# Meng-333/SRADSGAN

Measured on AMD Instinct MI355X. Metric: training images/sec (216x216, x4), higher is better.
Workload: dtype f32 (split-bf16 products: 3 bf16 MFMA terms per fp32 multiply, fp32 accumulate)

## Files before the change

### sradsgan_amd/csrc/conv_dev.h

```cpp
#pragma once
#include "conv_internal.h"

namespace srhip {

typedef unsigned int u32x4 __attribute__((ext_vector_type(4)));
typedef unsigned int u32x2 __attribute__((ext_vector_type(2)));
constexpr int FBK = 16;
constexpr int FLS = FBK + 4;
constexpr unsigned F_OOB = 0x80000000u;

struct FastGeom {
  int N, Hs, Ws, C, lds;
  int OH, OW, M;
  int ss;
  int TH, TW, dh0, dhs, dw0, dws;
  int kh0, khs, kw0, kws, KW;
  int Hd, Wd, dsd, ph, pw, ldd, K;
  int ldw, ldr;
  float slope;
  int flags, accumulate, dst_identity;
  unsigned src_bytes, w_bytes;
  int src_pp = 0, dst_pp = 0, src_guard = 0, dst_guard = 0;
  unsigned src_plane_bytes = 0, dst_plane_bytes = 0;
  void* dst2_pp = nullptr;
  int dst2_guard = 0;
  const float* res2 = nullptr;
  const float* res3 = nullptr;
};
struct ResRequest {
  const float* r2 = nullptr;
  const float* r3 = nullptr;
  int served = 0;
};
extern thread_local ResRequest g_res_req;
struct SignRequest {
  void* words = nullptr;
  size_t bytes = 0;
  int mode = 0;
  int served = 0;
};
extern thread_local SignRequest g_sign_req;
long pp_sign_tiles(int n, int h, int w, int cout);
struct PhaseSet {
  int n = 0;
  int first[5] = {0, 0, 0, 0, 0};
  struct P {
    int ph, pw, OH, OW, kh0, kw0, TH, TW, dh0, dw0, M, nblk_m;
  } p[4];
};
struct PhaseRequest {
  PhaseSet ps;
  int active = 0, launched = 0;
};
extern thread_local PhaseRequest g_phase_req;
struct Dst2Request {
  void* pp = nullptr;
  int served = 0;
};
extern thread_local Dst2Request g_dst2_req;

}
extern int g_tail_dbg;
namespace srhip {
extern int g_fast_cfg;
extern int g_wgrad_cfg;
extern int g_fast_dynlds;
extern int g_fast_ablate;
extern int g_sgam_cfg;
extern int g_pers_grid;
extern int g_pers_abl;
extern int g_rowtap_addr;
extern int g_rowtap_pipe;
extern int g_patch_ks;
extern int g_pers_small;
extern int g_flat_blocks;
extern int g_flat_abl;
extern int g_flat_f32_k8;
extern int g_patch8;
extern int g_patch8_abl;
extern int g_phase_batch;
extern int g_headconv_rows;
extern int g_pool_epi_any;

enum FastCfg : int {
  FAST_CFG_FORCE_PATCH = -2,
  FAST_CFG_FORCE_DMA = -1,
  FAST_CFG_AUTO = 0,
  FAST_CFG_REG_128x128_K32 = 1,
  FAST_CFG_REG_64x128 = 2,
  FAST_CFG_REG_64x128_K32 = 3,
  FAST_CFG_REG_256x128 = 4,
  FAST_CFG_REG_128x128 = 5,
  FAST_CFG_REG_128x64_K32 = 6,
  FAST_CFG_REG_64x64 = 7,
  FAST_CFG_REG_128x64_4x1_K32 = 8,
  FAST_CFG_REG_ONLY = 20,
  FAST_CFG_NO_PATCH = 21,
  FAST_CFG_NO_VALU = 22,
  FAST_CFG_PATCH_TO_DMA = 23,
  FAST_CFG_PATCH_NARROW = 24,
};
inline bool fast_cfg_allows_dma(int cfg) { return cfg < 1 || cfg == FAST_CFG_PATCH_TO_DMA || cfg == FAST_CFG_PATCH_NARROW; }

enum WgradCfg : int {
  WGRAD_CFG_AUTO = 0,
  WGRAD_CFG_BN64 = 1,
  WGRAD_CFG_BN128 = 2,
  WGRAD_CFG_BK32 = 3,
  WGRAD_CFG_BK32_BN64 = 4,
  WGRAD_CFG_TILE256 = 5,
  WGRAD_CFG_SCALAR_REDUCE_GENERIC = 6,
  WGRAD_CFG_NO_ROWTAP = 7,
  WGRAD_CFG_SCALAR_REDUCE = 8,
  WGRAD_CFG_NO_PAIRED_TAILS = 9,
  WGRAD_CFG_REG = 10,
  WGRAD_CFG_ROWTAP_TARGET = 100,
};

constexpr int FAST_EPI_MASK = 0x3f;
constexpr int FAST_ABL_NO_LOADS = 0x100;
constexpr int FAST_ABL_NO_BARRIER = 0x200;
constexpr int FAST_ABL_TIMING = FAST_ABL_NO_LOADS | FAST_ABL_NO_BARRIER;
constexpr int FAST_ABL_PLAIN_STORES = 0x400;

inline bool bytes_ok(long pixels, int ld, int c, unsigned* out) {
  const long b = pixels > 0 ? ((pixels - 1) * (long)ld + c) * 4L : 0;
  if (b >= (1L << 31)) return false;
  *out = (unsigned)b;
  return true;
}

__device__ inline float4 bufload4(__amdgpu_buffer_rsrc_t r, unsigned byte_off) {
  u32x4 v = __builtin_amdgcn_raw_buffer_load_b128(r, byte_off, 0, 0);
  return __builtin_bit_cast(float4, v);
}

__device__ inline f32x16 mfma32f(float a, float b, f32x16 c) {
  return __builtin_amdgcn_mfma_f32_32x32x2f32(a, b, c, 0, 0, 0);
}

__device__ inline int xcd_tile(int b, int nblk) {
  const int q = nblk >> 3, r = nblk & 7, x = b & 7;
  return (x < r ? x * (q + 1) : r * (q + 1) + (x - r) * q) + (b >> 3);
}

typedef __bf16 bf16x8_t __attribute__((ext_vector_type(8)));

__device__ inline void split_bf16x8(const float4& v0, const float4& v1, bf16x8_t& hi, bf16x8_t& lo) {
  const float v[8] = {v0.x, v0.y, v0.z, v0.w, v1.x, v1.y, v1.z, v1.w};
#pragma unroll
  for (int j = 0; j < 8; ++j) {
    const __bf16 h = (__bf16)v[j];
    hi[j] = h;
    lo[j] = (__bf16)(v[j] - (float)h);
  }
}

typedef _Float16 f16x8_t __attribute__((ext_vector_type(8)));
template <int PROD>
__device__ __forceinline__ f32x16 mma16(const bf16x8_t& a, const bf16x8_t& b, const f32x16& c) {
  if constexpr (PROD == 2)
    return __builtin_amdgcn_mfma_f32_32x32x16_f16(__builtin_bit_cast(f16x8_t, a), __builtin_bit_cast(f16x8_t, b), c, 0, 0, 0);
  else
    return __builtin_amdgcn_mfma_f32_32x32x16_bf16(a, b, c, 0, 0, 0);
}
template <int PROD>
__device__ __forceinline__ bf16x8_t round16x8(const float4& v0, const float4& v1) {
  const float v[8] = {v0.x, v0.y, v0.z, v0.w, v1.x, v1.y, v1.z, v1.w};
  if constexpr (PROD == 2) {
    f16x8_t h;
#pragma unroll
    for (int j = 0; j < 8; ++j) h[j] = (_Float16)v[j];
    return __builtin_bit_cast(bf16x8_t, h);
  } else {
    bf16x8_t h;
#pragma unroll
    for (int j = 0; j < 8; ++j) h[j] = (__bf16)v[j];
    return h;
  }
}
template <int PROD>
constexpr int nprod() { return PROD == 0 ? 3 : 1; }

__device__ inline void lds_dma16(const float* gsrc, unsigned lds_dst_uniform) {
  unsigned keep;
  asm volatile(
      "s_mov_b32 %0, m0\n\ts_mov_b32 m0, %2\n\ts_nop 0\n\tglobal_load_lds_dwordx4 %1, off\n\ts_mov_b32 m0, %0"
      : "=&s"(keep)
      : "v"(gsrc), "s"(lds_dst_uniform)
      : "memory");
}

__device__ inline void lds_dma16_buf(unsigned voff, __amdgpu_buffer_rsrc_t r, unsigned lds_dst_uniform) {
  asm volatile("s_mov_b32 m0, %2\n\ts_nop 0\n\tbuffer_load_dwordx4 %0, %1, 0 offen lds" ::"v"(voff), "s"(r), "s"(lds_dst_uniform) : "memory");
}

struct PatchGeom {
  int PH, PW, tiles_h, tiles_w;
  int PWP, PR, npieces;
  int lo_h, lo_w;
  unsigned gmap;
};

template <int N>
__device__ inline void wait_vmcnt() {
  asm volatile("s_waitcnt vmcnt(%0)" ::"n"(N) : "memory");
}

template <int I>
struct IC {
  static constexpr int value = I;
};

__device__ __forceinline__ void patch_pixel(int r, int PH, int PW, unsigned gmap, int& orow, int& ocol) {
  const int a = PW >> 4, b = PW & 15;
  const int grp = (gmap >> (4 * (r >> 4))) & 15, j = r & 15;
  const int nfull = PH * a;
  if (grp < nfull) {
    orow = grp / a;
    ocol = (grp - orow * a) * 16 + j;
  } else if (b > 0) {
    const int idx = (grp - nfull) * 16 + j;
    orow = idx / b;
    ocol = 16 * a + (idx - orow * b);
    if (orow >= PH) { orow = PH; ocol = 0; }
  } else {
    orow = PH;
    ocol = 0;
  }
}

struct PoolRequest {
  float* out = nullptr;
  unsigned sec_bytes = 0;
  int served_nseg = 0;
};
extern thread_local PoolRequest g_pool_req;
int launch_patch_pers(const float* src, const float* wt, const float* bias, const float* residual, const float* actmask,
                      float* dst, const FastGeom& g, const PatchGeom& pg, int nbm, int nbn, bool wide, int prod, int eflags,
                      hipStream_t st);

int launch_patch8(const float* src, const float* wt, const float* bias, const float* actmask, float* dst, const FastGeom& g,
                  const PatchGeom& pg, int nbm, int eflags, hipStream_t st);

}
```

### sradsgan_amd/csrc/conv_fast_fprop.hip

```cpp
#include "conv_dev.h"

namespace srhip {

int g_fast_ablate = 0;


template <int BM, int BN, int WM, int WN, int BK, int MATH = 0>
__global__ __launch_bounds__(WM* WN * 64) void fast_conv_kernel(const float* __restrict__ src,
                                                                 const float* __restrict__ wt,
                                                                 const float* __restrict__ bias,
                                                                 const float* __restrict__ residual,
                                                                 const float* __restrict__ rowscale,
                                                                 const float* __restrict__ chanscale,
                                                                 const float* __restrict__ actmask,
                                                                 float* __restrict__ dst, FastGeom g, int nblk_m,
                                                                 int nblk_n) {
  constexpr int NT = WM * WN * 64;
  constexpr int WTM = BM / WM, WTN = BN / WN;
  constexpr int TM = WTM / 32, TN = WTN / 32;
  constexpr int LS = BK + 4;
  constexpr int QPR = BK / 4;
  constexpr int RPP = NT / QPR;
  constexpr int AR = (BM + RPP - 1) / RPP, BR = (BN + RPP - 1) / RPP;
  constexpr int STAGE = (BM + BN) * LS;
// ... 1352 lines not shown
      r.wide = g.K >= 128;
      r.nbn = cdiv(g.K, r.wide ? 128 : 64);
      r.try_patch8 = r.wide && !a.residual;
      r.try_pers = true;
    }
    return r;
  }
  const bool valu_ok = cfg != FAST_CFG_REG_ONLY && cfg != FAST_CFG_NO_VALU &&
                       !(g.flags & ~(SRHIP_EPI_BIAS | SRHIP_EPI_LRELU | SRHIP_EPI_GRADDATA)) && !g.accumulate;
  if (g.K <= 4 && valu_ok && g.TH == 3 && g.TW == 3 && g.ss == 1 && g.dsd == 1 && g.ph == 0 && g.pw == 0 && g.Hd == g.OH && g.Wd == g.OW &&
      (g.dhs == 1 || g.dhs == -1) && (g.dws == 1 || g.dws == -1) && g.M >= 65536) {
    r.family = FpropFamily::Narrow;
    r.nd = g.K == 3 ? 3 : 4;
    return r;
  }
  if (g.K == 1 && g.C % 4 == 0 && g.lds % 4 == 0 && aligned16(a.src) && aligned16(a.wt) && g.M < 65536 && valu_ok) {
    r.family = FpropFamily::Dot;
    return r;
  }
  const int math16 = g_conv_math == 2 ? ((g.flags & SRHIP_EPI_GRADDATA) ? 2 : 3) : 1;
  if (g.K <= 32) {
    static const RegLaunch small[4] = {launch_reg<128, 32, 4, 1, 16>, launch_reg<128, 32, 4, 1, 16, 1>, launch_reg<128, 32, 4, 1, 16, 2>,
                                       launch_reg<128, 32, 4, 1, 16, 3>};
    r.family = FpropFamily::Reg;
    if (g_conv_math >= 1 && cfg != FAST_CFG_REG_ONLY && !(g.flags & (SRHIP_EPI_CHANSCALE | FAST_ABL_TIMING))) r.math = math16;
    r.reg = small[r.math];
    return r;
  }
  const bool al16 = g.K % 4 == 0 && g.ldd % 4 == 0 && aligned16(a.dst) && (!a.residual || (g.ldr % 4 == 0 && aligned16(a.residual))) &&
                    aligned16(a.actmask) && aligned16(a.bias);
  const bool dma_ok = fast_cfg_allows_dma(cfg) && !(g.flags & FAST_ABL_TIMING) && g.K >= 64 && al16;
  bool patch_to_dma = false;
  if (dma_ok && g_conv_math >= 1 && cfg != FAST_CFG_NO_PATCH && !scaled_a && !g.accumulate && plan_patch(g, &r.pg)) {
    r.nbm = g.N * r.pg.tiles_h * r.pg.tiles_w;
    r.wide = g.K >= 128 && cfg != FAST_CFG_PATCH_NARROW;
    r.bn = r.wide ? 128 : 64;
    r.nbn = cdiv(g.K, r.bn);
    const bool enough = (long)r.nbm * r.nbn >= 256;
    if (cfg == FAST_CFG_PATCH_TO_DMA) {
      patch_to_dma = enough;
    } else if (enough || cfg == FAST_CFG_FORCE_PATCH) {
      r.family = FpropFamily::Patch;
      r.math = math16;
      r.try_pers = !(g.flags & FAST_ABL_PLAIN_STORES);
      r.try_patch8 = r.try_pers && r.wide && math16 == 1 && !a.residual;
      r.ks = math16 == 1 && !r.wide && g_patch_ks && g.C % 32 == 0 && g.C >= 32;
      r.epi = math16 != 1 ? -1 : epi_variant(r.eflags, false);
      if (r.ks && r.epi != 0 && r.epi != SRHIP_EPI_BIAS && r.epi != SRHIP_EPI_RESIDUAL) r.epi = -1;
      return r;
    }
  }
  if (dma_ok && (!(r.eflags & SRHIP_EPI_CHANSCALE) || aligned16(a.chanscale))) {
    r.nbm = cdiv(g.M, 128);
    const bool force = cfg == FAST_CFG_FORCE_DMA || patch_to_dma;
    const long min_tiles = g_conv_math >= 1 ? 128 : 512;
    r.wide = g.K >= 128 && ((long)r.nbm * cdiv(g.K, 128) >= min_tiles || force);
    if (r.wide || (long)r.nbm * cdiv(g.K, 64) >= min_tiles || force) {
      r.family = FpropFamily::Dma;
      r.bn = r.wide ? 128 : 64;
      r.nbn = cdiv(g.K, r.bn);
      r.math = g_conv_math >= 1 ? math16 : 0;
      r.epi = (r.math >= 2 || g.accumulate) ? -1 : epi_variant(r.eflags, true);
      return r;
    }
  }
  struct Forced { int cfg; bool k128, k32; RegLaunch fn; };
  static const Forced forced[] = {
      {FAST_CFG_REG_128x128_K32, true, true, launch_reg<128, 128, 2, 2, 32>}, {FAST_CFG_REG_64x128, true, false, launch_reg<64, 128, 1, 4, 16>},
      {FAST_CFG_REG_64x128_K32, true, true, launch_reg<64, 128, 1, 4, 32>},   {FAST_CFG_REG_256x128, true, false, launch_reg<256, 128, 4, 2, 16>},
      {FAST_CFG_REG_128x128, true, false, launch_reg<128, 128, 2, 2, 16>},    {FAST_CFG_REG_128x64_K32, false, true, launch_reg<128, 64, 2, 2, 32>},
      {FAST_CFG_REG_64x64, false, false, launch_reg<64, 64, 2, 2, 16>},       {FAST_CFG_REG_128x64_4x1_K32, false, true, launch_reg<128, 64, 4, 1, 32>}};
  r.family = FpropFamily::Reg;
  const long b128 = (long)cdiv(g.M, 128) * cdiv(g.K, 128), b64 = (long)cdiv(g.M, 128) * cdiv(g.K, 64);
  r.reg = (g.K >= 128 && b128 >= 512) ? launch_reg<128, 128, 2, 2, 16> : b64 >= 512 ? launch_reg<128, 64, 2, 2, 16> : launch_reg<64, 64, 2, 2, 16>;
  for (const Forced& c : forced)
    if (cfg == c.cfg && (!c.k128 || g.K >= 128) && (!c.k32 || g.C % 32 == 0)) r.reg = c.fn;
  return r;
}

template <int BN, int EPI, int PROD = 0>
static int launch_patch(const ConvOperands& a, const FastGeom& g, const FpropRoute& r, hipStream_t st) {
  hipLaunchKernelGGL((conv_patch_kernel<BN, EPI, PROD>), dim3(r.nbm * r.nbn), dim3(256), 0, st, a.src, weight_section(a, g, PROD + 1), a.bias,
                     a.residual, a.actmask, a.dst, g, r.pg, r.nbm, r.nbn);
  return check_launch("conv_patch");
}
template <int EPI>
static int launch_patch_ks(const ConvOperands& a, const FastGeom& g, const FpropRoute& r, hipStream_t st) {
  hipLaunchKernelGGL((conv_patch_ks_kernel<EPI>), dim3(r.nbm * r.nbn), dim3(256), 0, st, a.src, weight_section(a, g, 1), a.bias, a.residual,
                     a.actmask, a.dst, g, r.pg, r.nbm, r.nbn);
  return check_launch("conv_patch_ks");
}
template <int BN, int EPI, int MATH>
static int launch_dma(const ConvOperands& a, const FastGeom& g, const FpropRoute& r, hipStream_t st) {
  PhaseSet ps;
  int grid = r.nbm * r.nbn;
  if constexpr (MATH <= 1) {
    if (g.dst2_pp) g_dst2_req.served = 1;
    if (g_phase_req.active) {
      ps = g_phase_req.ps;
      grid = 0;
      for (int k = 0; k < ps.n; ++k) {
        ps.first[k] = grid;
        grid += ps.p[k].nblk_m * r.nbn;
      }
      ps.first[ps.n] = grid;
      g_phase_req.launched = 1;
    }
  }
  hipLaunchKernelGGL((fast_conv_dma_kernel<128, BN, EPI, MATH>), dim3(grid), dim3(256), g_fast_dynlds, st, a.src, weight_section(a, g, MATH),
                     a.bias, a.residual, a.rowscale, a.chanscale, a.actmask, a.dst, g, r.nbm, r.nbn, ps);
  return check_launch("fast_conv_dma");
}
template <bool TAIL, class F>
static int with_epi(int epi, F f) {
  switch (epi) {
    case 0: return f(IC<0>{});
    case 1: return f(IC<1>{});
    case 3: return f(IC<3>{});
    case 32: return f(IC<32>{});
    case 4: return f(IC<4>{});
    case 29: if constexpr (TAIL) return f(IC<29>{}); [[fallthrough]];
    default: return f(IC<-1>{});
  }
}

static int launch_fprop(const ConvOperands& a, const FastGeom& g, const FpropRoute& r, hipStream_t st) {
  const bool wide = r.bn == 128;
  switch (r.family) {
    case FpropFamily::Nothing:
      return SRHIP_OK;
    case FpropFamily::Planes:
    case FpropFamily::Patch: {
      if (r.try_patch8) {
        const int rc8 = launch_patch8(a.src, a.wt, a.bias, a.actmask, a.dst, g, r.pg, r.nbm, r.eflags, st);
        if (rc8 >= 0) return rc8;
      }
      if (r.try_pers) {
        const int rc = launch_patch_pers(a.src, a.wt, a.bias, a.residual, a.actmask, a.dst, g, r.pg, r.nbm, r.nbn, r.wide, r.math - 1, r.eflags, st);
        if (rc >= 0) return rc;
      }
      if (r.family == FpropFamily::Planes) break;
      if (r.math == 2) return wide ? launch_patch<128, -1, 1>(a, g, r, st) : launch_patch<64, -1, 1>(a, g, r, st);
      if (r.math == 3) return wide ? launch_patch<128, -1, 2>(a, g, r, st) : launch_patch<64, -1, 2>(a, g, r, st);
      if (wide) return with_epi<false>(r.epi, [&](auto e) { return launch_patch<128, decltype(e)::value>(a, g, r, st); });
      if (!r.ks) return with_epi<false>(r.epi, [&](auto e) { return launch_patch<64, decltype(e)::value>(a, g, r, st); });
      switch (r.epi) {
        case 0: return launch_patch_ks<0>(a, g, r, st);
        case 1: return launch_patch_ks<1>(a, g, r, st);
        case 4: return launch_patch_ks<4>(a, g, r, st);
        default: return launch_patch_ks<-1>(a, g, r, st);
      }
    }
    case FpropFamily::Narrow: {
      const int th = cdiv(g.OH, 16), tw = cdiv(g.OW, 16);
      const int lo_h = g.dhs > 0 ? g.dh0 : g.dh0 + 2 * g.dhs, lo_w = g.dws > 0 ? g.dw0 : g.dw0 + 2 * g.dws;
      auto k = r.nd == 3 ? narrow_conv_kernel<3> : narrow_conv_kernel<4>;
      hipLaunchKernelGGL(k, dim3(g.N * th * tw), dim3(256), 0, st, a.src, a.wt, a.bias, a.dst, g, th, tw, lo_h, lo_w);
      return check_launch("narrow_conv");
    }
    case FpropFamily::Dot:
      hipLaunchKernelGGL(dot_conv_kernel, dim3(cdiv(g.M, 4)), dim3(256), 0, st, a.src, a.wt, a.bias, a.dst, g);
      return check_launch("dot_conv");
    case FpropFamily::Dma:
      if (r.math == 2) return wide ? launch_dma<128, -1, 2>(a, g, r, st) : launch_dma<64, -1, 2>(a, g, r, st);
      if (r.math == 3) return wide ? launch_dma<128, -1, 3>(a, g, r, st) : launch_dma<64, -1, 3>(a, g, r, st);
      if (r.math == 1 && wide) return with_epi<true>(r.epi, [&](auto e) { return launch_dma<128, decltype(e)::value, 1>(a, g, r, st); });
      if (r.math == 1) return with_epi<true>(r.epi, [&](auto e) { return launch_dma<64, decltype(e)::value, 1>(a, g, r, st); });
      if (wide) return with_epi<true>(r.epi, [&](auto e) { return launch_dma<128, decltype(e)::value, 0>(a, g, r, st); });
      return with_epi<true>(r.epi, [&](auto e) { return launch_dma<64, decltype(e)::value, 0>(a, g, r, st); });
    case FpropFamily::Reg:
      return r.reg(a, g, st);
  }
  set_error("conv2d (padded planes): shape / arithmetic mode not served by the persistent patch kernel");
  return SRHIP_ERR_ARG;
}

static int run_fast(const ConvOperands& a, const FastGeom& g, hipStream_t st) { return launch_fprop(a, g, choose_fprop_route(g, a), st); }

int fast_conv2d_fwd(const float* x, const float* packed, const float* bias, const float* residual,
                    const float* rowscale, const float* chanscale, float* y, int n, int h, int w, int cin, int cout, int kh, int kw,
                    int stride, int pad, int ldx, int ldy, int ldr, float slope, int flags, hipStream_t st) {
  SRHIP_REQUIRE(ldx % 4 == 0 && (((uintptr_t)x | (uintptr_t)packed) & 15) == 0, "conv2d_fwd: x/packed must be 16-byte aligned with ldx % 4 == 0");
  FastGeom g;
  g.N = n; g.Hs = h; g.Ws = w; g.C = cin; g.lds = ldx;
  g.OH = (h + 2 * pad - kh) / stride + 1;
  g.OW = (w + 2 * pad - kw) / stride + 1;
  SRHIP_REQUIRE(g.OH > 0 && g.OW > 0, "conv2d_fwd: empty output");
  const long M = (long)n * g.OH * g.OW;
  SRHIP_REQUIRE(M < (1L << 31), "conv2d_fwd: pixel count overflows int32");
  g.M = (int)M; g.ss = stride;
  g.TH = kh; g.TW = kw; g.dh0 = -pad; g.dhs = 1; g.dw0 = -pad; g.dws = 1;
  g.kh0 = 0; g.khs = 1; g.kw0 = 0; g.kws = 1; g.KW = kw;
  g.Hd = g.OH; g.Wd = g.OW; g.dsd = 1; g.ph = 0; g.pw = 0; g.ldd = ldy; g.K = cout;
  g.ldw = kh * kw * cin; g.ldr = ldr; g.slope = slope; g.flags = flags | g_fast_ablate; g.accumulate = 0; g.dst_identity = 1;
  SRHIP_REQUIRE(bytes_ok((long)n * h * w, ldx, cin, &g.src_bytes), "conv2d_fwd: source tensor >= 2 GiB");
  g.w_bytes = (unsigned)((long)cout * g.ldw * 4);
  if (g_dst2_req.pp != nullptr && stride == 1 && cout % 8 == 0 && g.OH == g.Hd && g.OW == g.Wd) {
    g.dst2_pp = g_dst2_req.pp;
    g.dst2_guard = pp_guard(g.Wd);
  }
  return run_fast({x, packed, bias, residual, rowscale, chanscale, nullptr, y}, g, st);
}

int fast_conv2d_fwd_pp(const void* x, int x_pp, const float* packed, const float* bias, void* y, int y_pp, int n, int h, int w, int cin,
                       int cout, int ldx, int ldy, float slope, int flags, hipStream_t st) {
  FastGeom g;
  g.N = n; g.Hs = h; g.Ws = w; g.C = cin; g.lds = x_pp ? cin : ldx;
  g.OH = h; g.OW = w;
  const long M = (long)n * h * w;
  SRHIP_REQUIRE(M < (1L << 31), "conv2d_fwd_pp: pixel count overflows int32");
  g.M = (int)M; g.ss = 1;
  g.TH = 3; g.TW = 3; g.dh0 = -1; g.dhs = 1; g.dw0 = -1; g.dws = 1;
  g.kh0 = 0; g.khs = 1; g.kw0 = 0; g.kws = 1; g.KW = 3;
  g.Hd = h; g.Wd = w; g.dsd = 1; g.ph = 0; g.pw = 0; g.ldd = y_pp ? cout : ldy; g.K = cout;
  g.ldw = 9 * cin; g.ldr = 0; g.slope = slope; g.flags = flags; g.accumulate = 0; g.dst_identity = 1;
  const long ppx = pp_plane_pixels(n, h, w);
  g.src_pp = x_pp; g.dst_pp = y_pp;
  g.src_guard = g.dst_guard = pp_guard(w);
  if (x_pp) {
    SRHIP_REQUIRE(ppx * cin * 4L < (1L << 31), "conv2d_fwd_pp: source planes >= 2 GiB");
    g.src_plane_bytes = (unsigned)(ppx * cin * 2L);
    g.src_bytes = 2u * g.src_plane_bytes;
  } else {
    SRHIP_REQUIRE(bytes_ok(M, ldx, cin, &g.src_bytes), "conv2d_fwd_pp: source tensor >= 2 GiB");
  }
  if (y_pp) {
    SRHIP_REQUIRE(ppx * cout * 4L < (1L << 31), "conv2d_fwd_pp: destination planes >= 2 GiB");
    g.dst_plane_bytes = (unsigned)(ppx * cout * 2L);
  }
  g.w_bytes = (unsigned)((long)cout * g.ldw * 4);
  return run_fast({static_cast<const float*>(x), packed, bias, nullptr, nullptr, nullptr, nullptr, static_cast<float*>(y)}, g, st);
}

int fast_conv2d_dgrad_pp(const void* dy, int dy_pp, const float* packed, void* dx, int dx_pp, const float* residual, const void* actmask,
                         float slope, int n, int h, int w, int cin, int cout, int ldy, int ldx, int ldr, hipStream_t st) {
  FastGeom g;
  g.N = n; g.Hs = h; g.Ws = w; g.C = cout; g.lds = dy_pp ? cout : ldy;
  g.KW = 3; g.Hd = h; g.Wd = w; g.dsd = 1; g.ldd = dx_pp ? cin : ldx; g.K = cin;
  g.ldw = 9 * cout; g.ldr = ldr; g.slope = slope; g.accumulate = 0;
  g.flags = (residual ? SRHIP_EPI_RESIDUAL : 0) | (actmask ? SRHIP_EPI_ACTMASK : 0) | SRHIP_EPI_GRADDATA;
  g.ss = 1; g.dhs = -1; g.dws = -1; g.khs = 1; g.kws = 1;
  g.dst_identity = 1;
  g.ph = 0; g.pw = 0; g.OH = h; g.OW = w; g.kh0 = 0; g.kw0 = 0;
  g.TH = 3; g.TW = 3;
  g.dh0 = 1; g.dw0 = 1;
  const long M = (long)n * h * w;
  SRHIP_REQUIRE(M < (1L << 31), "conv2d_dgrad_pp: pixel count overflows int32");
  g.M = (int)M;
  const long ppx = pp_plane_pixels(n, h, w);
  g.src_pp = dy_pp; g.dst_pp = dx_pp;
  g.src_guard = g.dst_guard = pp_guard(w);
  if (dy_pp) {
    SRHIP_REQUIRE(ppx * cout * 4L < (1L << 31), "conv2d_dgrad_pp: dy planes >= 2 GiB");
    g.src_plane_bytes = (unsigned)(ppx * cout * 2L);
    g.src_bytes = 2u * g.src_plane_bytes;
  } else {
    SRHIP_REQUIRE(bytes_ok(M, ldy, cout, &g.src_bytes), "conv2d_dgrad_pp: dy tensor >= 2 GiB");
  }
  if (dx_pp) {
    SRHIP_REQUIRE(ppx * cin * 4L < (1L << 31), "conv2d_dgrad_pp: dx planes >= 2 GiB");
    g.dst_plane_bytes = (unsigned)(ppx * cin * 2L);
  }
  g.w_bytes = (unsigned)((long)cin * g.ldw * 4);
  if (residual && !dx_pp) {
    g.res2 = g_res_req.r2;
    g.res3 = g_res_req.r3;
  }
  return run_fast({static_cast<const float*>(dy), packed, nullptr, residual, nullptr, nullptr, static_cast<const float*>(actmask),
                   static_cast<float*>(dx)}, g, st);
}

int fast_conv2d_dgrad(const float* dy, const float* packed, float* dx, const float* residual, const float* actmask,
                      float slope, int n, int h, int w, int cin, int cout, int kh, int kw, int stride, int pad, int ldy,
                      int ldx, int ldr, int accumulate, hipStream_t st) {
  SRHIP_REQUIRE(ldy % 4 == 0 && (((uintptr_t)dy | (uintptr_t)packed) & 15) == 0, "conv2d_dgrad: dy/packed must be 16-byte aligned with ldy % 4 == 0");
  const int ho = (h + 2 * pad - kh) / stride + 1, wo = (w + 2 * pad - kw) / stride + 1;
  SRHIP_REQUIRE(ho > 0 && wo > 0, "conv2d_dgrad: empty dy");
  FastGeom g;
  g.N = n; g.Hs = ho; g.Ws = wo; g.C = cout; g.lds = ldy;
  g.KW = kw; g.Hd = h; g.Wd = w; g.dsd = stride; g.ldd = ldx; g.K = cin;
  g.ldw = kh * kw * cout; g.ldr = ldr; g.slope = slope; g.accumulate = accumulate ? 1 : 0;
  g.flags = (residual ? SRHIP_EPI_RESIDUAL : 0) | (actmask ? SRHIP_EPI_ACTMASK : 0) | SRHIP_EPI_GRADDATA;
  g.ss = 1; g.dhs = -1; g.dws = -1; g.khs = stride; g.kws = stride;
  g.dst_identity = stride == 1 ? 1 : 0;
  SRHIP_REQUIRE(bytes_ok((long)n * ho * wo, ldy, cout, &g.src_bytes), "conv2d_dgrad: dy tensor >= 2 GiB");
  g.w_bytes = (unsigned)((long)cin * g.ldw * 4);
  if (residual && stride == 1 && !accumulate) {
    g.res2 = g_res_req.r2;
    g.res3 = g_res_req.r3;
  }
  PhaseRequest& pq = g_phase_req;
  pq = PhaseRequest();
  if (stride == 2 && g_conv_math != 2 && g_phase_batch) {
    bool all = true;
    int k = 0;
    for (int ph = 0; ph < stride && all; ++ph)
      for (int pw = 0; pw < stride && all; ++pw) {
        PhaseSet::P& q = pq.ps.p[k++];
        q.ph = ph; q.pw = pw;
        q.OH = (h - ph + stride - 1) / stride;
        q.OW = (w - pw + stride - 1) / stride;
        q.kh0 = (ph + pad) % stride; q.kw0 = (pw + pad) % stride;
        q.TH = q.kh0 < kh ? (kh - q.kh0 + stride - 1) / stride : 0;
        q.TW = q.kw0 < kw ? (kw - q.kw0 + stride - 1) / stride : 0;
        q.dh0 = (ph + pad - q.kh0) / stride; q.dw0 = (pw + pad - q.kw0) / stride;
        const long M = (long)n * q.OH * q.OW;
// ... 36 lines not shown
```

### sradsgan_amd/csrc/conv_igemm.hip

```cpp
#include "common.h"

namespace srhip {
int g_headconv_rows = 4;
}
namespace srhip {

constexpr int BK = 16;

struct ConvGeom {
  int N, H, W, C;
  int Ho, Wo, K;
  int KH, KW;
  int so, pad, dv;
  int ldx, ldy, ldr, ldw;
  int Ktot;
  int M;
  float slope;
  int flags;
  int accumulate;
};

__device__ inline f32x16 mfma32(float a, float b, f32x16 c) {
  return __builtin_amdgcn_mfma_f32_32x32x2f32(a, b, c, 0, 0, 0);
}

template <int BM, int BN, int WM, int WN, bool VEC>
__global__ __launch_bounds__(256) void igemm_fprop_kernel(const float* __restrict__ src,
                                                           const float* __restrict__ wt,
                                                           const float* __restrict__ bias,
                                                           const float* __restrict__ residual,
                                                           const float* __restrict__ rowscale,
                                                           float* __restrict__ dst, ConvGeom g) {
  constexpr int WTM = BM / WM, WTN = BN / WN;
  constexpr int TM = WTM / 32, TN = WTN / 32;
  constexpr int LDA = BM + 2, LDB = BN + 4;
  constexpr int AR = BM / 64;
  constexpr int BVEC = BK * BN / 4;
  constexpr int BV = (BVEC + 255) / 256;
  __shared__ __attribute__((aligned(16))) float lds[2 * BK * LDA + 2 * BK * LDB];
  float* As = lds;
  float* Bs = lds + 2 * BK * LDA;

  const int tid = threadIdx.x;
  const int ntn = (g.K + BN - 1) / BN;
  const int tile_n = blockIdx.x % ntn;
  const int tile_m = blockIdx.x / ntn;
  const int m0 = tile_m * BM, n0 = tile_n * BN;

  const int arow = tid >> 2, kq = tid & 3;
  int hb[AR], wb[AR], pb[AR];
  const int HoWo = g.Ho * g.Wo;
#pragma unroll
  for (int i = 0; i < AR; ++i) {
    int m = m0 + arow + 64 * i;
    if (m < g.M) {
      int n = m / HoWo;
      int rem = m - n * HoWo;
      int ho = rem / g.Wo;
      int wo = rem - ho * g.Wo;
      hb[i] = ho * g.so - g.pad;
      wb[i] = wo * g.so - g.pad;
      pb[i] = n * g.H * g.W;
    } else {
      hb[i] = -(1 << 28);
      wb[i] = 0;
      pb[i] = 0;
    }
  }

  float4 ra[AR];
  float4 rb[BV];

  auto gather1 = [&](int i, int k) -> float {
    if (k >= g.Ktot) return 0.f;
    int tap = k / g.C;
    int c = k - tap * g.C;
    int kh = tap / g.KW;
    int kw = tap - kh * g.KW;
    int hn = hb[i] + kh, wn = wb[i] + kw;
    if (hn < 0 || wn < 0) return 0.f;
    int hs = hn, ws = wn;
    if (g.dv > 1) {
      hs = hn / g.dv;
      ws = wn / g.dv;
      if (hs * g.dv != hn || ws * g.dv != wn) return 0.f;
    }
    if (hs >= g.H || ws >= g.W) return 0.f;
    return src[(size_t)(pb[i] + hs * g.W + ws) * g.ldx + c];
  };

  auto load_tiles = [&](int kc) {
    const int k = kc * BK + kq * 4;
    if (VEC) {
      int tap = k / g.C;
      int c = k - tap * g.C;
      int kh = tap / g.KW;
      int kw = tap - kh * g.KW;
      const bool kok = k < g.Ktot;
#pragma unroll
      for (int i = 0; i < AR; ++i) {
        int hn = hb[i] + kh, wn = wb[i] + kw;
        bool ok = kok && hn >= 0 && wn >= 0;
        int hs = hn, ws = wn;
        if (g.dv > 1) {
          hs = hn / g.dv;
          ws = wn / g.dv;
          ok = ok && (hs * g.dv == hn) && (ws * g.dv == wn);
        }
        ok = ok && hs < g.H && ws < g.W;
        ra[i] = ok ? *reinterpret_cast<const float4*>(src + (size_t)(pb[i] + hs * g.W + ws) * g.ldx + c)
                   : make_float4(0.f, 0.f, 0.f, 0.f);
      }
    } else {
#pragma unroll
      for (int i = 0; i < AR; ++i) {
        ra[i].x = gather1(i, k);
        ra[i].y = gather1(i, k + 1);
        ra[i].z = gather1(i, k + 2);
        ra[i].w = gather1(i, k + 3);
      }
    }
#pragma unroll
    for (int j = 0; j < BV; ++j) {
      int idx = tid + 256 * j;
      int brow = idx / (BN / 4), bc = idx - brow * (BN / 4);
      int kk = kc * BK + brow, col = n0 + bc * 4;
      bool ok = (BVEC % 256 == 0 || idx < BVEC) && kk < g.Ktot && col < g.ldw;
      rb[j] = ok ? *reinterpret_cast<const float4*>(wt + (size_t)kk * g.ldw + col)
                 : make_float4(0.f, 0.f, 0.f, 0.f);
    }
  };

  auto store_tiles = [&](int buf) {
    float* a = As + buf * BK * LDA + (kq * 4) * LDA + arow;
#pragma unroll
    for (int i = 0; i < AR; ++i) {
      a[0 * LDA + 64 * i] = ra[i].x;
      a[1 * LDA + 64 * i] = ra[i].y;
      a[2 * LDA + 64 * i] = ra[i].z;
      a[3 * LDA + 64 * i] = ra[i].w;
    }
#pragma unroll
    for (int j = 0; j < BV; ++j) {
      int idx = tid + 256 * j;
      if (BVEC % 256 == 0 || idx < BVEC) {
        int brow = idx / (BN / 4), bc = idx - brow * (BN / 4);
        *reinterpret_cast<float4*>(Bs + buf * BK * LDB + brow * LDB + bc * 4) = rb[j];
      }
    }
  };

  const int lane = tid & 63, wave = tid >> 6;
  const int wm = wave / WN, wn = wave - wm * WN;
// ... 576 lines not shown
  WgradPlan p;
  p.bm = cout > 64 ? 128 : (cout > 32 ? 64 : 32);
  p.bn = p.bm == 32 ? 128 : 64;
  long tiles = (long)cdiv(cout, p.bm) * cdiv(ktot, p.bn);
  int nchunks = cdiv(M, BK);
  long want = (1024 + tiles - 1) / tiles;
  if (cout <= 4 && want < 256) want = 256;
  long maxsplit = (nchunks + 15) / 16;
  long ns = want < 1 ? 1 : want;
  if (ns > maxsplit) ns = maxsplit;
  if (ns < 1) ns = 1;
  p.chunks_per_split = (int)((nchunks + ns - 1) / ns);
  p.nsplit = cdiv(nchunks, p.chunks_per_split);
  return p;
}

}

namespace srhip {

int legacy_packed_ld(int cdst) { return ((cdst + 31) / 32) * 32; }

int legacy_pack_weight(const float* w, float* packed, int cout, int cin, int kh, int kw, int mode, void* stream) {
  SRHIP_REQUIRE(w && packed && cout > 0 && cin > 0 && kh > 0 && kw > 0 && (mode == 0 || mode == 1),
                "pack_weight: bad argument");
  int csrc = mode == 0 ? cin : cout, cdst = mode == 0 ? cout : cin;
  int ld = legacy_packed_ld(cdst);
  long total = (long)kh * kw * csrc * ld;
  hipLaunchKernelGGL(pack_weight_kernel, dim3(cdiv(total, 256)), dim3(256), 0, as_stream(stream), w, packed, cout,
                     cin, kh, kw, mode, ld);
  return check_launch("pack_weight");
}

int legacy_conv2d_fwd(const float* x, const float* packed, const float* bias, const float* residual,
                     const float* rowscale, float* y, int n, int h, int w, int cin, int cout, int kh, int kw,
                     int stride, int pad, int ldx, int ldy, int ldr, float slope, int flags, void* stream) {
  SRHIP_REQUIRE(x && packed && y, "conv2d_fwd: null tensor");
  SRHIP_REQUIRE(n >= 0 && h > 0 && w > 0 && cin > 0 && cout > 0 && kh > 0 && kw > 0 && stride > 0 && pad >= 0,
                "conv2d_fwd: bad geometry");
  SRHIP_REQUIRE(ldx >= cin && ldy >= cout, "conv2d_fwd: row stride smaller than channel count");
  SRHIP_REQUIRE(!(flags & SRHIP_EPI_BIAS) || bias, "conv2d_fwd: EPI_BIAS without bias");
  SRHIP_REQUIRE(!(flags & SRHIP_EPI_RESIDUAL) || (residual && ldr >= cout), "conv2d_fwd: EPI_RESIDUAL without residual");
  SRHIP_REQUIRE(!(flags & SRHIP_EPI_ROWSCALE) || rowscale, "conv2d_fwd: EPI_ROWSCALE without rowscale");
  ConvGeom g;
  g.N = n; g.H = h; g.W = w; g.C = cin;
  g.Ho = (h + 2 * pad - kh) / stride + 1;
  g.Wo = (w + 2 * pad - kw) / stride + 1;
  SRHIP_REQUIRE(g.Ho > 0 && g.Wo > 0, "conv2d_fwd: empty output");
  g.K = cout; g.KH = kh; g.KW = kw; g.so = stride; g.pad = pad; g.dv = 1;
  g.ldx = ldx; g.ldy = ldy; g.ldr = ldr; g.ldw = legacy_packed_ld(cout);
  g.Ktot = kh * kw * cin;
  long M = (long)n * g.Ho * g.Wo;
  SRHIP_REQUIRE(M < (1L << 31) && (long)n * h * w < (1L << 31), "conv2d_fwd: pixel count overflows int32");
  g.M = (int)M; g.slope = slope; g.flags = flags; g.accumulate = 0;
  if (cin <= 3 && kh == 3 && kw == 3 && stride == 1 && pad == 1 && M >= 65536 &&
      !(flags & ~(SRHIP_EPI_BIAS | SRHIP_EPI_LRELU)) && (size_t)3 * (w + 2) * cin * sizeof(float) <= 32 * 1024) {
    const int rpb = g_headconv_rows > 0 ? g_headconv_rows : 1;
    hipLaunchKernelGGL(headconv_fwd_kernel, dim3(cdiv((long)n * h, rpb), cdiv(cout, 64)), dim3(256), (size_t)3 * (w + 2) * cin * sizeof(float),
                       as_stream(stream), x, packed, bias, y, n, h, w, cin, cout, ldx, ldy, g.ldw, slope, flags, rpb);
    return check_launch("headconv_fwd");
  }
  return run_fprop(x, packed, bias, residual, rowscale, y, g, as_stream(stream));
}

int legacy_conv2d_dgrad(const float* dy, const float* packed, float* dx, int n, int h, int w, int cin, int cout,
                       int kh, int kw, int stride, int pad, int ldy, int ldx, int accumulate, void* stream) {
  SRHIP_REQUIRE(dy && packed && dx, "conv2d_dgrad: null tensor");
  SRHIP_REQUIRE(n >= 0 && h > 0 && w > 0 && cin > 0 && cout > 0 && kh > 0 && kw > 0 && stride > 0 && pad >= 0,
                "conv2d_dgrad: bad geometry");
  SRHIP_REQUIRE(pad <= kh - 1 && pad <= kw - 1, "conv2d_dgrad: pad > kernel-1 unsupported");
  SRHIP_REQUIRE(ldy >= cout && ldx >= cin, "conv2d_dgrad: row stride smaller than channel count");
  ConvGeom g;
  g.N = n;
  g.H = (h + 2 * pad - kh) / stride + 1;
  g.W = (w + 2 * pad - kw) / stride + 1;
  SRHIP_REQUIRE(g.H > 0 && g.W > 0, "conv2d_dgrad: empty dy");
  g.C = cout; g.Ho = h; g.Wo = w; g.K = cin; g.KH = kh; g.KW = kw;
  g.so = 1; g.pad = kh - 1 - pad; g.dv = stride;
  SRHIP_REQUIRE(kh == kw, "conv2d_dgrad: square kernels only");
  g.ldx = ldy; g.ldy = ldx; g.ldr = 0; g.ldw = legacy_packed_ld(cin);
  g.Ktot = kh * kw * cout;
  long M = (long)n * h * w;
  SRHIP_REQUIRE(M < (1L << 31), "conv2d_dgrad: pixel count overflows int32");
  g.M = (int)M; g.slope = 0.f; g.flags = 0; g.accumulate = accumulate ? 1 : 0;
  return run_fprop(dy, packed, nullptr, nullptr, nullptr, dx, g, as_stream(stream));
}

size_t legacy_conv2d_wgrad_workspace(int n, int h, int w, int cin, int cout, int kh, int kw, int stride, int pad) {
  int ho = (h + 2 * pad - kh) / stride + 1, wo = (w + 2 * pad - kw) / stride + 1;
  long M = (long)n * ho * wo;
  if (M <= 0) return 0;
  WgradPlan p = plan_wgrad((int)M, cout, kh * kw * cin);
  return (size_t)p.nsplit * cout * kh * kw * cin * sizeof(float);
}

size_t legacy_conv2d_wgrad_bias_workspace(int n, int h, int w, int cin, int cout, int kh, int kw, int stride, int pad) {
  const int ho = (h + 2 * pad - kh) / stride + 1, wo = (w + 2 * pad - kw) / stride + 1;
  const long M = (long)n * ho * wo;
  if (M <= 0) return 0;
  return (size_t)plan_wgrad((int)M, cout, kh * kw * cin).nsplit * cout * sizeof(float);
}

int legacy_conv2d_wgrad(const float* x, const float* dy, float* dw, void* workspace, size_t workspace_bytes, int n,
                       int h, int w, int cin, int cout, int kh, int kw, int stride, int pad, int ldx, int ldy,
                       void* stream, float* db, float* bias_ws, int* bias_done, const float* ymask, float slope) {
  if (bias_done) *bias_done = 0;
  SRHIP_REQUIRE(!ymask || (db && bias_ws && bias_done && cin <= 3 && kh == 3 && kw == 3 && stride == 1 && pad == 1 &&
                           (long)n * h * w >= 65536 && (size_t)3 * (w + 2) * cin * sizeof(float) <= 32 * 1024),
                "conv2d_wgrad: the fused activation mask is built for the 3-channel 3x3 head convs at full image size (with bias)");
  SRHIP_REQUIRE(x && dy && dw, "conv2d_wgrad: null tensor");
  SRHIP_REQUIRE(n > 0 && h > 0 && w > 0 && cin > 0 && cout > 0 && kh > 0 && kw > 0 && stride > 0 && pad >= 0,
                "conv2d_wgrad: bad geometry");
  SRHIP_REQUIRE(ldx >= cin && ldy >= cout, "conv2d_wgrad: row stride smaller than channel count");
  ConvGeom g;
  g.N = n; g.H = h; g.W = w; g.C = cin;
  g.Ho = (h + 2 * pad - kh) / stride + 1;
  g.Wo = (w + 2 * pad - kw) / stride + 1;
  SRHIP_REQUIRE(g.Ho > 0 && g.Wo > 0, "conv2d_wgrad: empty output");
  g.K = cout; g.KH = kh; g.KW = kw; g.so = stride; g.pad = pad; g.dv = 1;
  g.ldx = ldx; g.ldy = ldy; g.ldr = 0; g.ldw = 0; g.Ktot = kh * kw * cin;
  long M = (long)n * g.Ho * g.Wo;
  SRHIP_REQUIRE(M < (1L << 31) && (long)n * h * w < (1L << 31), "conv2d_wgrad: pixel count overflows int32");
  g.M = (int)M; g.slope = 0.f; g.flags = 0; g.accumulate = 0;
  WgradPlan p = plan_wgrad(g.M, cout, g.Ktot);
  size_t need = (size_t)p.nsplit * cout * g.Ktot * sizeof(float);
  if (!workspace || workspace_bytes < need) {
    set_error("conv2d_wgrad: workspace %zu bytes < required %zu", workspace_bytes, need);
    return SRHIP_ERR_WORKSPACE;
  }
  float* partial = static_cast<float*>(workspace);
  hipStream_t st = as_stream(stream);
  if (cin <= 3 && kh == 3 && kw == 3 && stride == 1 && pad == 1 && g.M >= 65536 &&
      (size_t)3 * (w + 2) * cin * sizeof(float) <= 32 * 1024) {
    const int rows = n * h;
    int ns = p.nsplit < rows ? p.nsplit : rows;
    const int rps = cdiv(rows, ns);
    ns = cdiv(rows, rps);
    const bool fuse_bias = db != nullptr && bias_ws != nullptr && bias_done != nullptr;
    hipLaunchKernelGGL(wgrad_smallcin_kernel, dim3(ns, cdiv(cout, 64)), dim3(256), (size_t)32 * 1024, st,
                       x, dy, ymask, slope, partial, fuse_bias ? bias_ws : nullptr, n, h, w, cin, cout, ldx, ldy, rps);
    int rc0 = check_launch("wgrad_smallcin");
    if (rc0) return rc0;
    long total0 = (long)cout * g.Ktot;
    hipLaunchKernelGGL(wgrad_reduce_kernel, dim3(cdiv(total0, 16)), dim3(256), 0, st, partial, dw, ns, cout, cin, kh * kw,
                       g.Ktot);
    if (fuse_bias) {
      hipLaunchKernelGGL(wgrad_reduce_kernel, dim3(cdiv(cout, 16)), dim3(256), 0, st, bias_ws, db, ns, cout, 1, 1, 1);
      *bias_done = 1;
    }
    return check_launch("wgrad_reduce");
  }
  if (cout <= 4 && cin % 64 == 0 && ldx % 4 == 0 && ((uintptr_t)x & 15) == 0 && kh == 3 && kw == 3 && stride == 1 && pad == 1 &&
      g.M >= 65536 && p.nsplit >= 64) {
    const int th = cdiv(h, 16), tw = cdiv(w, 16);
    const int ns = p.nsplit < 256 ? p.nsplit : 256;
    const size_t lds_bytes = (size_t)(18 * 18 * 64 + 256 * 4) * sizeof(float);
#define SRHIP_WN(ND_)                                                                                                    \
  do {                                                                                                                   \
    static bool attr_set = false;                                                                                        \
    if (!attr_set) {                                                                                                     \
      (void)hipFuncSetAttribute(reinterpret_cast<const void*>(wgrad_narrow_kernel<ND_>),                                 \
                                hipFuncAttributeMaxDynamicSharedMemorySize, (int)lds_bytes);                             \
      attr_set = true;                                                                                                   \
    }                                                                                                                    \
    hipLaunchKernelGGL(wgrad_narrow_kernel<ND_>, dim3(ns, cin / 64), dim3(576), lds_bytes, st, x, dy, partial, n, h, w,  \
                       cin, ldx, ldy, th, tw);                                                                           \
  } while (0)
    if (cout == 1) SRHIP_WN(1);
    else if (cout == 2) SRHIP_WN(2);
    else if (cout == 3) SRHIP_WN(3);
    else SRHIP_WN(4);
#undef SRHIP_WN
    int rc1 = check_launch("wgrad_narrow");
    if (rc1) return rc1;
    hipLaunchKernelGGL(wgrad_reduce_kernel, dim3(cdiv((long)cout * g.Ktot, 16)), dim3(256), 0, st, partial, dw, ns, cout, cin,
                       kh * kw, g.Ktot);
    return check_launch("wgrad_reduce");
  }
  const bool va = (cout % 4 == 0) && (ldy % 4 == 0);
  const bool vb = (cin % 4 == 0) && (ldx % 4 == 0);
  int rc;
  if (p.bm == 128)
    rc = launch_wgrad<128, 64, 2, 2>(x, dy, partial, g, p.nsplit, p.chunks_per_split, va, vb, st);
  else if (p.bm == 64)
    rc = launch_wgrad<64, 64, 2, 2>(x, dy, partial, g, p.nsplit, p.chunks_per_split, va, vb, st);
  else
    rc = launch_wgrad<32, 128, 1, 4>(x, dy, partial, g, p.nsplit, p.chunks_per_split, va, vb, st);
  if (rc) return rc;
  long total = (long)cout * g.Ktot;
  hipLaunchKernelGGL(wgrad_reduce_kernel, dim3(cdiv(total, 16)), dim3(256), 0, st, partial, dw, p.nsplit, cout, cin,
                     kh * kw, g.Ktot);
  return check_launch("wgrad_reduce");
}

}
```

Baseline: 678.0.

## Add tap-matrix MFMA kernels for narrow-output conv forward and weight gradient

Adds new kernels for convolutions with very few output channels (3 or 4, e.g. the final RGB conv). The forward pass computes per-tap partial products as a GEMM with N=9*Cout using fp32 MFMA, then sums the shifted taps from LDS. The weight gradient is treated the same way, building a tap-expanded dy matrix so that MFMA reduces over pixels. These paths become the default and replace the VALU narrow kernels, which stay reachable through a config flag. The aim is to avoid the poor MFMA use of tiny-N GEMMs, at the cost of more LDS traffic and an extra shifted-sum epilogue.

```diff
diff --git a/sradsgan_amd/csrc/conv_dev.h b/sradsgan_amd/csrc/conv_dev.h
--- a/sradsgan_amd/csrc/conv_dev.h
+++ b/sradsgan_amd/csrc/conv_dev.h
@@ -58,6 +58,10 @@
   int served = 0;
 };
 extern thread_local Dst2Request g_dst2_req;
+
+int launch_narrow_tap(const float* src, const float* wt, const float* bias, float* dst, const FastGeom& g, int nd, hipStream_t st);
+int launch_wgrad_narrow_tap(const float* x, const float* dy, float* partial, int n, int h, int w, int cin, int cout, int ldx, int ldy,
+                            int ns_max, int* ns_out, hipStream_t st);
 
 }
 extern int g_tail_dbg;
@@ -99,8 +103,9 @@
   FAST_CFG_NO_VALU = 22,
   FAST_CFG_PATCH_TO_DMA = 23,
   FAST_CFG_PATCH_NARROW = 24,
-};
-inline bool fast_cfg_allows_dma(int cfg) { return cfg < 1 || cfg == FAST_CFG_PATCH_TO_DMA || cfg == FAST_CFG_PATCH_NARROW; }
+  FAST_CFG_NARROW_VALU = 25,
+};
+inline bool fast_cfg_allows_dma(int cfg) { return cfg < 1 || cfg == FAST_CFG_PATCH_TO_DMA || cfg == FAST_CFG_PATCH_NARROW || cfg == FAST_CFG_NARROW_VALU; }
 
 enum WgradCfg : int {
   WGRAD_CFG_AUTO = 0,
diff --git a/sradsgan_amd/csrc/conv_fast_fprop.hip b/sradsgan_amd/csrc/conv_fast_fprop.hip
--- a/sradsgan_amd/csrc/conv_fast_fprop.hip
+++ b/sradsgan_amd/csrc/conv_fast_fprop.hip
@@ -1528,6 +1528,7 @@
       }
     }
     case FpropFamily::Narrow: {
+      if (g_fast_cfg != FAST_CFG_NARROW_VALU) return launch_narrow_tap(a.src, a.wt, a.bias, a.dst, g, r.nd, st);
       const int th = cdiv(g.OH, 16), tw = cdiv(g.OW, 16);
       const int lo_h = g.dhs > 0 ? g.dh0 : g.dh0 + 2 * g.dhs, lo_w = g.dws > 0 ? g.dw0 : g.dw0 + 2 * g.dws;
       auto k = r.nd == 3 ? narrow_conv_kernel<3> : narrow_conv_kernel<4>;
diff --git a/sradsgan_amd/csrc/conv_igemm.hip b/sradsgan_amd/csrc/conv_igemm.hip
--- a/sradsgan_amd/csrc/conv_igemm.hip
+++ b/sradsgan_amd/csrc/conv_igemm.hip
@@ -1,4 +1,4 @@
-#include "common.h"
+#include "conv_dev.h"
 
 namespace srhip {
 int g_headconv_rows = 4;
@@ -881,6 +881,14 @@
   }
   if (cout <= 4 && cin % 64 == 0 && ldx % 4 == 0 && ((uintptr_t)x & 15) == 0 && kh == 3 && kw == 3 && stride == 1 && pad == 1 &&
       g.M >= 65536 && p.nsplit >= 64) {
+    if (g_fast_cfg != FAST_CFG_NARROW_VALU) {
+      int nst = 0;
+      const int rct = launch_wgrad_narrow_tap(x, dy, partial, n, h, w, cin, cout, ldx, ldy, p.nsplit, &nst, st);
+      if (rct) return rct;
+      hipLaunchKernelGGL(wgrad_reduce_kernel, dim3(cdiv((long)cout * g.Ktot, 16)), dim3(256), 0, st, partial, dw, nst, cout, cin,
+                         kh * kw, g.Ktot);
+      return check_launch("wgrad_reduce");
+    }
     const int th = cdiv(h, 16), tw = cdiv(w, 16);
     const int ns = p.nsplit < 256 ? p.nsplit : 256;
     const size_t lds_bytes = (size_t)(18 * 18 * 64 + 256 * 4) * sizeof(float);
diff --git a/sradsgan_amd/csrc/conv_narrow.hip b/sradsgan_amd/csrc/conv_narrow.hip
--- /dev/null
+++ b/sradsgan_amd/csrc/conv_narrow.hip
@@ -0,0 +1,304 @@
+#include "conv_dev.h"
+
+namespace srhip {
+
+template <int ND, int CK>
+__global__ __launch_bounds__(256, 2) void narrow_tap_kernel(const float* __restrict__ src, const float* __restrict__ wt,
+                                                             const float* __restrict__ bias, float* __restrict__ dst, FastGeom g,
+                                                             int nstrips, int sw, int rsplit, int rb, int lo_h, int lo_w) {
+  constexpr int NCOL = 9 * ND, NT = (NCOL + 31) / 32;
+  constexpr int SP = 64;
+  constexpr int TP = 68;
+  constexpr int QP = CK / 4;
+  constexpr int HQ = CK / 8;
+  constexpr int NLD = 2 * SP * QP / 256;
+  constexpr int NPASS = (2 * ND * 64 + 255) / 256;
+  extern __shared__ __attribute__((aligned(16))) float smem[];
+  float4* xs = reinterpret_cast<float4*>(smem);
+  float* tr = smem + 2 * SP * CK;
+  const int tid = threadIdx.x, lane = tid & 63;
+  const int wave = __builtin_amdgcn_readfirstlane(tid >> 6);
+  const int l31 = lane & 31, half = lane >> 5;
+  const int mt = wave & 1, wrow = wave >> 1;
+
+  int b = blockIdx.x;
+  const int rs = b % rsplit;
+  b /= rsplit;
+  const int strip = b % nstrips, img = b / nstrips;
+  const int q0 = rs * rb;
+  const int nrows = min(rb, g.OH - q0);
+  const int ow0 = strip * sw;
+  const int swv = min(sw, g.OW - ow0);
+  if (nrows <= 0 || swv <= 0) return;
+  const int nch = g.C / CK;
+  const int nit = (nrows + 3) >> 1;
+
+  int scol[NLD];
+  int sdst[NLD];
+#pragma unroll
+  for (int i = 0; i < NLD; ++i) {
+    const int e = tid + i * 256;
+    const int q = e % QP, pix = (e / QP) % SP, rsel = e / (QP * SP);
+    const int sc = ow0 + lo_w + pix;
+    scol[i] = (pix < swv + 2 && sc >= 0 && sc < g.Ws) ? sc * g.lds + q * 4 : -1;
+    sdst[i] = (rsel * SP + pix) * QP + (q ^ (pix & (QP - 1)));
+  }
+  float4 stage[NLD];
+  auto fetch = [&](int it, int cc) {
+#pragma unroll
+    for (int i = 0; i < NLD; ++i) {
+      const int rsel = (tid + i * 256) / (QP * SP);
+      const int sh = q0 + lo_h + 2 * it + rsel;
+      stage[i] = make_float4(0.f, 0.f, 0.f, 0.f);
+      if (scol[i] >= 0 && sh >= 0 && sh < g.Hs)
+        stage[i] = *reinterpret_cast<const float4*>(src + (size_t)(img * g.Hs + sh) * g.Ws * g.lds + scol[i] + cc * CK);
+    }
+  };
+
+  float bw[NT][CK / 2];
+  const float* wcol[NT];
+#pragma unroll
+  for (int t = 0; t < NT; ++t) {
+    const int col = t * 32 + l31;
+    const int tap = col / ND, co = col - tap * ND;
+    const int th = tap / 3, tw = tap - th * 3;
+    wcol[t] = (col < NCOL && co < g.K)
+                  ? wt + (size_t)co * g.ldw + (size_t)((g.kh0 + th * g.khs) * g.KW + (g.kw0 + tw * g.kws)) * g.C + half * (CK / 2)
+                  : nullptr;
+  }
+  auto load_weights = [&](int cc) {
+#pragma unroll
+    for (int t = 0; t < NT; ++t)
+#pragma unroll
+      for (int v = 0; v < CK / 8; ++v) {
+        const float4 w4 = wcol[t] ? *reinterpret_cast<const float4*>(wcol[t] + cc * CK + v * 4) : make_float4(0.f, 0.f, 0.f, 0.f);
+        bw[t][v * 4 + 0] = w4.x;
+        bw[t][v * 4 + 1] = w4.y;
+        bw[t][v * 4 + 2] = w4.z;
+        bw[t][v * 4 + 3] = w4.w;
+      }
+  };
+  if (nch == 1) load_weights(0);
+
+  const int ah0 = g.dh0 - lo_h, aw0 = g.dw0 - lo_w;
+  const int pi = mt * 32 + l31;
+  const float4* arow = xs + (wrow * SP + pi) * QP;
+
+  f32x16 acc[NT];
+  fetch(0, 0);
+  for (int it = 0; it < nit; ++it) {
+    for (int cc = 0; cc < nch; ++cc) {
+      if (cc != 0) __syncthreads();
+#pragma unroll
+      for (int i = 0; i < NLD; ++i) xs[sdst[i]] = stage[i];
+      __syncthreads();
+      if (cc + 1 < nch) fetch(it, cc + 1);
+      else if (it + 1 < nit) fetch(it + 1, 0);
+      if (nch > 1) load_weights(cc);
+      if (cc == 0) {
+#pragma unroll
+        for (int t = 0; t < NT; ++t)
+#pragma unroll
+          for (int r = 0; r < 16; ++r) acc[t][r] = 0.f;
+      }
+      float4 av[HQ];
+#pragma unroll
+      for (int v = 0; v < HQ; ++v) av[v] = arow[(half * HQ + v) ^ (pi & (QP - 1))];
+#pragma unroll
+      for (int v = 0; v < HQ; ++v) {
+#pragma unroll
+        for (int t = 0; t < NT; ++t) {
+          acc[t] = mfma32f(av[v].x, bw[t][v * 4 + 0], acc[t]);
+          acc[t] = mfma32f(av[v].y, bw[t][v * 4 + 1], acc[t]);
+          acc[t] = mfma32f(av[v].z, bw[t][v * 4 + 2], acc[t]);
+          acc[t] = mfma32f(av[v].w, bw[t][v * 4 + 3], acc[t]);
+        }
+      }
+    }
+    {
+      const int slot = (2 * it + wrow) & 3;
+#pragma unroll
+      for (int t = 0; t < NT; ++t) {
+        const int col = t * 32 + l31;
+        if (col < NCOL) {
+          float* tcol = tr + (slot * NCOL + col) * TP + mt * 32 + 4 * half;
+#pragma unroll
+          for (int gq = 0; gq < 4; ++gq)
+            *reinterpret_cast<float4*>(tcol + 8 * gq) = make_float4(acc[t][4 * gq], acc[t][4 * gq + 1], acc[t][4 * gq + 2], acc[t][4 * gq + 3]);
+        }
+      }
+    }
+    __syncthreads();
+#pragma unroll
+    for (int k = 0; k < NPASS; ++k) {
+      const int e = tid + k * 256;
+      const int px = e & 63, grp = e >> 6;
+      const int osel = grp / ND, co = grp - osel * ND;
+      const int o = 2 * it - 2 + osel;
+      if (e < 2 * ND * 64 && o >= 0 && o < nrows && px < swv && co < g.K) {
+        float s = 0.f;
+#pragma unroll
+        for (int th = 0; th < 3; ++th) {
+          const int slot = (o + ah0 + th * g.dhs) & 3;
+#pragma unroll
+          for (int tw = 0; tw < 3; ++tw) {
+            const float v = tr[(slot * NCOL + (th * 3 + tw) * ND + co) * TP + px + aw0 + tw * g.dws];
+            s = (th == 0 && tw == 0) ? v : s + v;
+          }
+        }
+        if (g.flags & SRHIP_EPI_BIAS) s += bias[co];
+        if (g.flags & SRHIP_EPI_LRELU) s = s > 0.f ? s : s * g.slope;
+        dst[(((size_t)img * g.Hd + q0 + o) * g.Wd + ow0 + px) * g.ldd + co] = s;
+      }
+    }
+  }
+}
+
+template <int ND, int CK>
+static int launch_narrow_tap_as(const float* src, const float* wt, const float* bias, float* dst, const FastGeom& g, hipStream_t st) {
+  const int nstrips = cdiv(g.OW, 62), sw = cdiv(g.OW, nstrips);
+  int rsplit = cdiv(512, (long)g.N * nstrips);
+  if (rsplit > cdiv(g.OH, 16)) rsplit = cdiv(g.OH, 16);
+  if (rsplit < 1) rsplit = 1;
+  int rb = cdiv(g.OH, rsplit);
+  rb += rb & 1;
+  rsplit = cdiv(g.OH, rb);
+  const int lo_h = g.dhs > 0 ? g.dh0 : g.dh0 + 2 * g.dhs, lo_w = g.dws > 0 ? g.dw0 : g.dw0 + 2 * g.dws;
+  const size_t lds_bytes = (size_t)(2 * 64 * CK + 4 * 9 * ND * 68) * sizeof(float);
+  static bool attr_set = false;
+  if (!attr_set) {
+    (void)hipFuncSetAttribute(reinterpret_cast<const void*>(narrow_tap_kernel<ND, CK>), hipFuncAttributeMaxDynamicSharedMemorySize, (int)lds_bytes);
+    attr_set = true;
+  }
+  hipLaunchKernelGGL((narrow_tap_kernel<ND, CK>), dim3(g.N * nstrips * rsplit), dim3(256), lds_bytes, st, src, wt, bias, dst, g, nstrips, sw,
+                     rsplit, rb, lo_h, lo_w);
+  return check_launch("narrow_tap");
+}
+
+int launch_narrow_tap(const float* src, const float* wt, const float* bias, float* dst, const FastGeom& g, int nd, hipStream_t st) {
+  const bool c64 = g.C % 64 == 0;
+  if (nd == 3) return c64 ? launch_narrow_tap_as<3, 64>(src, wt, bias, dst, g, st) : launch_narrow_tap_as<3, 16>(src, wt, bias, dst, g, st);
+  return c64 ? launch_narrow_tap_as<4, 64>(src, wt, bias, dst, g, st) : launch_narrow_tap_as<4, 16>(src, wt, bias, dst, g, st);
+}
+
+template <int ND>
+__global__ __launch_bounds__(512) void wgrad_narrow_tap_kernel(const float* __restrict__ x, const float* __restrict__ dy,
+                                                                float* __restrict__ partial, int N, int H, int W, int cin, int ldx,
+                                                                int ldy, int nseg, int segw, int upb) {
+  constexpr int CAP = 128;
+  constexpr int NCOL = 9 * ND, NT = (NCOL + 31) / 32;
+  constexpr int DYE = 3 * (CAP + 2) * ND;
+  constexpr int NDL = (DYE + 511) / 512;
+  __shared__ __attribute__((aligned(16))) float xs[CAP * 64];
+  __shared__ float dys[DYE];
+  const int tid = threadIdx.x, lane = tid & 63;
+  const int wave = __builtin_amdgcn_readfirstlane(tid >> 6);
+  const int l31 = lane & 31, half = lane >> 5;
+  const int ci0 = blockIdx.y * 64;
+  const int units = N * H * nseg;
+  const int u_begin = blockIdx.x * upb, u_end = min(u_begin + upb, units);
+
+  int koff[NT];
+#pragma unroll
+  for (int t = 0; t < NT; ++t) {
+    const int col = t * 32 + l31;
+    const int tap = col / ND, co = col - tap * ND;
+    const int kh = tap / 3, kw = tap - kh * 3;
+    koff[t] = col < NCOL ? ((2 - kh) * (CAP + 2) + (2 - kw)) * ND + co : -1;
+  }
+  f32x16 acc[NT][2];
+#pragma unroll
+  for (int t = 0; t < NT; ++t)
+#pragma unroll
+    for (int r = 0; r < 16; ++r) acc[t][0][r] = acc[t][1][r] = 0.f;
+
+  float4 xst[4];
+  float dyst[NDL];
+  auto fetch = [&](int u) {
+    const int r = u / nseg, seg = u - r * nseg;
+    const int n = r / H, oh = r - n * H;
+    const int seg0 = seg * segw, width = min(segw, W - seg0);
+#pragma unroll
+    for (int i = 0; i < 4; ++i) {
+      const int e = tid + i * 512;
+      const int q = e & 15, t = e >> 4;
+      xst[i] = make_float4(0.f, 0.f, 0.f, 0.f);
+      if (t < width) xst[i] = *reinterpret_cast<const float4*>(x + ((size_t)r * W + seg0 + t) * ldx + ci0 + q * 4);
+    }
+#pragma unroll
+    for (int i = 0; i < NDL; ++i) {
+      const int e = tid + i * 512;
+      const int co = e % ND, bcol = (e / ND) % (CAP + 2), a = e / (ND * (CAP + 2));
+      const int ih = oh - 1 + a, iw = seg0 - 1 + bcol;
+      dyst[i] = 0.f;
+      if (e < DYE && bcol < width + 2 && ih >= 0 && ih < H && iw >= 0 && iw < W) dyst[i] = dy[((size_t)(n * H + ih) * W + iw) * ldy + co];
+    }
+  };
+  if (u_begin < u_end) fetch(u_begin);
+  for (int u = u_begin; u < u_end; ++u) {
+    const int seg = u % nseg;
+    const int width = min(segw, W - seg * segw);
+    __syncthreads();
+#pragma unroll
+    for (int i = 0; i < 4; ++i) *reinterpret_cast<float4*>(xs + (size_t)(tid + i * 512) * 4) = xst[i];
+#pragma unroll
+    for (int i = 0; i < NDL; ++i)
+      if (tid + i * 512 < DYE) dys[tid + i * 512] = dyst[i];
+    __syncthreads();
+    if (u + 1 < u_end) fetch(u + 1);
+    for (int kp = wave; 2 * kp < width; kp += 8) {
+      const int t = 2 * kp + half;
+      const float b0 = xs[t * 64 + l31], b1 = xs[t * 64 + 32 + l31];
+#pragma unroll
+      for (int tt = 0; tt < NT; ++tt) {
+        const float a = koff[tt] >= 0 ? dys[koff[tt] + t * ND] : 0.f;
+        acc[tt][0] = mfma32f(a, b0, acc[tt][0]);
+        acc[tt][1] = mfma32f(a, b1, acc[tt][1]);
+      }
+    }
+  }
+  float* red = xs;
+  for (int w = 0; w < 8; ++w) {
+    __syncthreads();
+    if (wave == w) {
+#pragma unroll
+      for (int t = 0; t < NT; ++t)
+#pragma unroll
+        for (int r = 0; r < 16; ++r) {
+          const int row = t * 32 + (r & 3) + 8 * (r >> 2) + 4 * half;
+          float* p0 = red + row * 64 + l31;
+          p0[0] = w == 0 ? acc[t][0][r] : p0[0] + acc[t][0][r];
+          p0[32] = w == 0 ? acc[t][1][r] : p0[32] + acc[t][1][r];
+        }
+    }
+  }
+  __syncthreads();
+  const int ktot = 9 * cin;
+  for (int e = tid; e < NCOL * 64; e += 512) {
+    const int c = e & 63, col = e >> 6;
+    const int tap = col / ND, co = col - tap * ND;
+    partial[(size_t)blockIdx.x * ND * ktot + (size_t)co * ktot + tap * cin + ci0 + c] = red[e];
+  }
+}
+
+int launch_wgrad_narrow_tap(const float* x, const float* dy, float* partial, int n, int h, int w, int cin, int cout, int ldx, int ldy,
+                            int ns_max, int* ns_out, hipStream_t st) {
+  const int nseg = cdiv(w, 128), segw = cdiv(w, nseg);
+  const long units = (long)n * h * nseg;
+  long want = ns_max < 256 ? ns_max : 256;
+  if (want > units) want = units;
+  const int upb = cdiv(units, want);
+  const int ns = cdiv(units, upb);
+  const dim3 grid(ns, cin / 64);
+#define SRHIP_WNT(ND_) \
+  hipLaunchKernelGGL(wgrad_narrow_tap_kernel<ND_>, grid, dim3(512), 0, st, x, dy, partial, n, h, w, cin, ldx, ldy, nseg, segw, upb)
+  if (cout == 1) SRHIP_WNT(1);
+  else if (cout == 2) SRHIP_WNT(2);
+  else if (cout == 3) SRHIP_WNT(3);
+  else SRHIP_WNT(4);
+#undef SRHIP_WNT
+  *ns_out = ns;
+  return check_launch("wgrad_narrow_tap");
+}
+
+}
```

Result: no change. 681.3 (median of 6 runs) (+0.5%).
